# sdrobert/pydrobert-speech

Hardware: AMD Instinct MI355X
Metric: frames/s (whole node) + HBM-roofline %, 40-mel fbank 16kHz 25/10ms (higher is better)
Workload: dtype f32

## Files before the change

pydrobert-speech_amd/csrc/pds_internal.h:

```cpp
#pragma once
#include <hip/hip_runtime.h>
#include <stdint.h>

#include <exception>
#include <new>
#include <string>

#include "../../include/pds_amd.h"

namespace pds {

void set_error(const std::string &msg);
int32_t hip_fail(hipError_t err, const char *what);

#define PDS_HIP(call)                                       \
  do {                                                      \
    hipError_t _e = (call);                                 \
    if (_e != hipSuccess) return pds::hip_fail(_e, #call);  \
  } while (0)

struct FastTables {
  int kind = 0;
  int n1 = 0, n2 = 0;
  int rows = 0;
  int num_cus = 0;
  float *d_window = nullptr;
  float *d_twiddle = nullptr;
  float *d_tw_special = nullptr;
  float *d_win_half = nullptr;
  float *d_tw_seed = nullptr;
  float *d_ell_w = nullptr;
  int32_t *d_ell_meta = nullptr;
  int32_t *d_ell_len = nullptr;
  int32_t *d_ell_woff = nullptr;
  int ell_wfloats = 0, ell_slots = 0;
  float *d_seg_w = nullptr;
  int32_t *d_seg_meta = nullptr;
  int seg_rounds = 0, seg_len = 0, seg_wfloats = 0, seg_meta_ints = 0;
  float *d_rs_w = nullptr;
  int32_t *d_rs_meta = nullptr;
  int rs_rounds = 0, rs_len = 0, rs_wfloats = 0;
  float *d_rsn_w = nullptr;
  int32_t *d_rsn_meta = nullptr;
  int rsn_rounds = 0, rsn_len = 0, rsn_wfloats = 0;
  int rs_eslot = -1;
  float *d_ms_w = nullptr;
  int32_t *d_ms_meta = nullptr;
  int ms_rounds = 0, ms_len = 0, ms_wfloats = 0, ms_meta_ints = 0, ms_slots = 0;
  long ms_reads = 0;
  int walk = 0;
  long rs_reads = 0, rs_cost = 0, ell_reads = 0, seg_reads = 0;
  float *d_mf_tab = nullptr;
  int mf_rows = 0;
};

}

struct pds_stft_plan {
  pds_stft_desc d;
  int device = 0;
  int num_bins = 0;
  float *d_window_f32 = nullptr;
  double *d_window_f64 = nullptr;
  int32_t *d_row_ptr = nullptr;
// ... 128 lines not shown
```

pydrobert-speech_amd/csrc/stft_fast.hip:

```cpp
#include "stft_wave_launch.h"

namespace pds {

#if PDS_STAMPS
unsigned long long *g_stamp_buf = nullptr;
extern "C" __attribute__((visibility("default"))) void pds_debug_set_stamp_buffer(unsigned long long *d_buf) {
  g_stamp_buf = d_buf;
}
#endif

extern "C" __attribute__((visibility("default"))) int32_t pds_build_experiments(void) { return PDS_EXPERIMENTS ? 1 : 0; }

bool fast_has_f64in(const pds_stft_plan *plan) { return plan->fast.kind && fast_f64in_kind(plan->fast.kind); }

bool fast_has_fused_cmvn(const pds_stft_plan *plan) {
  const FastTables &ft = plan->fast;
  return ft.kind && ft.n2 == 16 && ((ft.n1 == 64 && ft.walk != 0) || (ft.n1 == 32 && (ft.walk == 1 || ft.walk == 3)));
}

bool fast_has_fused_deltas(const pds_stft_plan *plan) {
  const FastTables &ft = plan->fast;
  return ft.kind && fast_deltas_kind(ft.kind) && ft.rsn_rounds >= 1 && ft.rsn_rounds <= 2 &&
         (!plan->d.include_energy || ft.rs_eslot >= 0);
}
// ... 157 lines not shown
        first[j] = (pstr - longest) & ~3;
      if (first[j] < 0) return PDS_OK;
      ell_meta[(size_t)sl * n2 + j] = first[j] | ((f + 1) << 16);
      if (f < 0) continue;
      for (int q = row_ptr[f]; q < row_ptr[f + 1]; ++q) {
        const int t = col[q] - first[j];
        if (t < 0 || t >= longest) return PDS_OK;
        ell_w[(size_t)ell_woff[sl] + (size_t)j * wstride + t] = (float)val[q];
      }
    }
  }
  if (ell_w.empty()) ell_w.assign(4, 0.0f);
  ft.ell_wfloats = (int)ell_w.size();
  ft.ell_slots = slots;
  int32_t rc = PDS_OK;
  const int groups = 64 / n2;
  bool dense_bank = false;
  long dense_reads = 0;
  if ((n2 == 16 || (pow2 && n2 >= 32)) && d.num_filts > 0 && d.num_filts <= 65535) {
    long ell_reads = 0;
    for (int sl = 0; sl < slots; ++sl) ell_reads += 2L * (ell_len[sl] / 4);
    ft.ell_reads = ell_reads;
    const int free_slots = (wave_area_floats(n1, n2) - groups * pstr) / groups;
    int best_len = 0, best_rounds = 0;
    long best_reads = 0, any_reads = 0;
    const char *only_len = std::getenv("PDS_SEG_LEN");
    for (int len : {16, 32, 64}) {
      if (only_len && std::atoi(only_len) != len) continue;
      long nseg = 0;
      for (int f = 0; f < d.num_filts; ++f) nseg += (span(f) + len - 1) / len;
// ... 33 lines not shown
          if (first < 0) ok = false;
          seg_meta[slot] = first;
          for (int q = row_ptr[f]; q < row_ptr[f + 1]; ++q) {
            if (col[q] < base + k * len || col[q] >= base + (k + 1) * len) continue;
            const int t = col[q] - first;
            if (t < 0 || t >= len) ok = false; else seg_w[(size_t)slot * wstride + t] = (float)val[q];
          }
        }
      }
      if (ok) {
        ft.seg_reads = best_reads;
        ft.seg_rounds = best_rounds;
        ft.seg_len = len;
        ft.seg_wfloats = (int)seg_w.size();
        ft.seg_meta_ints = (int)seg_meta.size();
        if (rc == PDS_OK) rc = upload(&ft.d_seg_w, seg_w.data(), seg_w.size());
        if (rc == PDS_OK) rc = upload(&ft.d_seg_meta, seg_meta.data(), seg_meta.size());
      }
    }
  }
  if (n2 == 16 && rc == PDS_OK) {
    RsegTables rs;
    const int area_floats = wave_area_floats(n1, n2);
    if (build_rseg(d.num_filts, row_ptr, col, val, N / 2 + 1, area_floats / 4, 8, rs)) {
      ft.rs_rounds = rs.rounds;
      ft.rs_len = rs.seg_len;
      ft.rs_wfloats = (int)rs.w.size();
      ft.rs_reads = rs.reads_per_lane();
      ft.rs_cost = rs.cost;
      RsegTables rn;
      ft.rs_eslot = -1;
      if (rc == PDS_OK && fast_deltas_kind(N) && build_rseg(d.num_filts, row_ptr, col, val, N / 2 + 1, area_floats / 4, 2, rn, true)) {
        ft.rsn_rounds = rn.rounds;
        ft.rsn_len = rn.seg_len;
        ft.rsn_wfloats = (int)rn.w.size();
        for (size_t at = 0; at < rn.meta.size() && ft.rs_eslot < 0; ++at)
          if ((rn.meta[at] >> 16) == 0) ft.rs_eslot = (int)at;
        rc = upload(&ft.d_rsn_w, rn.w.data(), rn.w.size());
        if (rc == PDS_OK) rc = upload(&ft.d_rsn_meta, rn.meta.data(), rn.meta.size());
      }
      if (rc == PDS_OK) rc = upload(&ft.d_rs_w, rs.w.data(), rs.w.size());
      if (rc == PDS_OK) rc = upload(&ft.d_rs_meta, rs.meta.data(), rs.meta.size());
    }
  }
  if (n2 == 16 && pow2 && rc == PDS_OK && dense_bank) {
    MsegTables ms;
    const int area_floats = wave_area_floats(n1, n2);
    const int max_slots = (area_floats - 4 * pstr) / 16;
    if (build_mseg(d.num_filts, row_ptr, col, val, pstr, max_slots, ms)) {
      ft.ms_rounds = ms.rounds;
      ft.ms_slots = ms.slots;
      ft.ms_len = ms.seg_len;
      ft.ms_wfloats = (int)ms.w.size();
      ft.ms_meta_ints = (int)ms.meta.size();
      ft.ms_reads = ms.reads_per_lane();
      rc = upload(&ft.d_ms_w, ms.w.data(), ms.w.size());
      if (rc == PDS_OK) rc = upload(&ft.d_ms_meta, ms.meta.data(), ms.meta.size());
    }
  }
  {
    const char *force = std::getenv("PDS_STFT_WALK");
    ft.walk = ft.seg_rounds > 0 ? 1 : 0;
    const bool ms_stands_in = ft.walk == 0 && dense_bank && ft.ms_rounds > 0 && N >= PDS_MSEG_MIN_N;
    const long other = ft.walk == 1 ? ft.seg_reads : ms_stands_in ? dense_reads : ft.ell_reads;
    if (ft.rs_rounds > 0 && 10 * ft.rs_reads <= 7 * other) ft.walk = 2;
    if (force && std::strcmp(force, "ell") == 0) ft.walk = 0;
    if (force && std::strcmp(force, "seg") == 0) ft.walk = ft.seg_rounds > 0 ? 1 : 0;
    if (force && std::strcmp(force, "rseg") == 0) ft.walk = ft.rs_rounds > 0 ? 2 : ft.walk;
    if ((ft.walk == 1 || (ft.walk == 0 && ms_stands_in)) && ft.ms_rounds > 0 && N >= PDS_MSEG_MIN_N && !force) ft.walk = 3;
    if (force && std::strcmp(force, "mseg") == 0 && ft.ms_rounds > 0) ft.walk = 3;
    if (std::getenv("PDS_DEBUG_PLAN"))
      std::fprintf(stderr,
                   "pds plan N=%d filters=%d: ell slots %d reads %ld | seg rounds %d len %d reads %ld | rseg rounds %d "
                   "len %d reads %ld cost %ld | mseg rounds %d len %d reads %ld -> walk %d\n",
                   N, d.num_filts, ft.ell_slots, ft.ell_reads, ft.seg_rounds, ft.seg_len, ft.seg_reads, ft.rs_rounds,
                   ft.rs_len, ft.rs_reads, ft.rs_cost, ft.ms_rounds, ft.ms_len, ft.ms_reads, ft.walk);
  }
  if (rc == PDS_OK) rc = upload(&ft.d_ell_w, ell_w.data(), ell_w.size());
  if (rc == PDS_OK) rc = upload(&ft.d_ell_meta, ell_meta.data(), ell_meta.size());
  if (rc == PDS_OK) rc = upload(&ft.d_ell_len, ell_len.data(), ell_len.size());
  if (rc == PDS_OK) rc = upload(&ft.d_ell_woff, ell_woff.data(), ell_woff.size());
  if (rc == PDS_OK) rc = upload(&ft.d_window, win.data(), win.size());
  if (rc == PDS_OK) rc = upload(&ft.d_twiddle, tw.data(), tw.size());
  if (((n1 == 32 || n1 == 64) && n2 == 16) || lean_geometry(n1, n2)) {
    std::vector<float> wh(win), seed((size_t)n2 * 6);
    for (float &v : wh) v *= PDS_RDFT_DIT ? 1.0f : 0.5f;
    const int mult[3] = {1, 4, n1 / 4};
    for (int r = 0; r < n2; ++r)
      for (int j = 0; j < 3; ++j) {
        const double ang = -2.0 * M_PI * (double)((r * mult[j]) % N) / (double)N;
        seed[((size_t)r * 3 + j) * 2 + 0] = (float)std::cos(ang);
        seed[((size_t)r * 3 + j) * 2 + 1] = (float)std::sin(ang);
      }
    if (rc == PDS_OK) rc = upload(&ft.d_win_half, wh.data(), wh.size());
    if (rc == PDS_OK) rc = upload(&ft.d_tw_seed, seed.data(), seed.size());
  }
  std::vector<float> tws((size_t)n2 * 2);
  for (int r = 0; r < n2; ++r) {
    const double ang = -2.0 * M_PI * (double)r / (double)(2 * n2);
    tws[2 * r] = (float)std::cos(ang);
    tws[2 * r + 1] = (float)std::sin(ang);
  }
  if (rc == PDS_OK) rc = upload(&ft.d_tw_special, tws.data(), tws.size());
  {
    const char *front = PDS_EXPERIMENTS ? std::getenv("PDS_STFT_FRONT") : nullptr;
    const int rows = (d.frame_length + n2 - 1) / n2;
    int bucket = 0;
    for (int b : {20, 25, 28, 30, 32})
      if (!bucket && rows <= b) bucket = b;
    MfmaFrontTables mt;
    if (rc == PDS_OK && n1 == 32 && n2 == 16 && bucket && front && std::strcmp(front, "mfma") == 0 &&
        build_mfma_front(n1, bucket, d.frame_length, window, mt)) {
      std::vector<float> image;
      image.reserve(mt.words());
      image.insert(image.end(), mt.win.begin(), mt.win.end());
      for (int32_t v : mt.off) {
        float f;
        std::memcpy(&f, &v, sizeof f);
// ... 10 lines not shown
  if (rc != PDS_OK) return rc;
  hipDeviceProp_t prop;
  PDS_HIP(hipGetDeviceProperties(&prop, plan->device));
  ft.num_cus = prop.multiProcessorCount;
  ft.n1 = n1;
  ft.n2 = n2;
  ft.rows = (d.frame_length + n2 - 1) / n2;
  ft.kind = d.dft_size;
  return PDS_OK;
}

void fast_tables_destroy(pds_stft_plan *plan) {
  FastTables &ft = plan->fast;
  (void)hipFree(ft.d_window);
  (void)hipFree(ft.d_twiddle);
  (void)hipFree(ft.d_tw_special);
  (void)hipFree(ft.d_win_half);
  (void)hipFree(ft.d_tw_seed);
  (void)hipFree(ft.d_mf_tab);
  (void)hipFree(ft.d_rs_w);
  (void)hipFree(ft.d_ms_w);
  (void)hipFree(ft.d_ms_meta);
  (void)hipFree(ft.d_rsn_w);
  (void)hipFree(ft.d_rsn_meta);
  (void)hipFree(ft.d_rs_meta);
  (void)hipFree(ft.d_seg_w);
  (void)hipFree(ft.d_seg_meta);
  (void)hipFree(ft.d_ell_w);
  (void)hipFree(ft.d_ell_meta);
  (void)hipFree(ft.d_ell_len);
  (void)hipFree(ft.d_ell_woff);
  ft = FastTables();
}

}
```

pydrobert-speech_amd/csrc/stft_switches.h:

```cpp
#pragma once
namespace pds {

#ifndef PDS_PRIO_PACK
#define PDS_PRIO_PACK 0x103212
#endif
#if PDS_PRIO_PACK == 0xffffff
#define PDS_PHASE(i) __builtin_amdgcn_sched_barrier(0)
#else
#define PDS_PHASE(i) do { if (PDS_PRIO_PACK >= 0) __builtin_amdgcn_s_setprio(((PDS_PRIO_PACK) >> (4 * (i))) & 3); } while (0)
#endif
#ifndef PDS_ABLATE
#define PDS_ABLATE 0
#endif
#ifndef PDS_STAMPS
#define PDS_STAMPS 0
#endif
#if PDS_STAMPS
extern unsigned long long *g_stamp_buf;
#define PDS_STAMP(i, drain)                                               \
  do {                                                                    \
    if (PDS_STAMPS == 2) break;                                           \
    __builtin_amdgcn_sched_barrier(0);                                    \
    if (drain) asm volatile("s_waitcnt vmcnt(0)" ::: "memory");           \
    const unsigned long long now_ = __builtin_readcyclecounter();         \
// ... 6 lines not shown
#endif
#ifndef PDS_SEG_DEEP_N
#define PDS_SEG_DEEP_N 1024
#endif
#ifndef PDS_ELL_DEEP_N
#define PDS_ELL_DEEP_N 4096
#endif
#ifndef PDS_MSEG_MIN_N
#define PDS_MSEG_MIN_N 1024
#endif
#ifndef PDS_PAIR_SPLIT
#define PDS_PAIR_SPLIT 1
#endif
#ifndef PDS_N4096_MINW
#define PDS_N4096_MINW 2
#endif
#ifndef PDS_FAST_PROLOGUE
#define PDS_FAST_PROLOGUE 1
#endif
#ifndef PDS_MSEG_RED4
#define PDS_MSEG_RED4 1
#endif
#ifndef PDS_FILTER_UNROLL
#define PDS_FILTER_UNROLL 2
#endif
#ifndef PDS_EXPERIMENTS
#define PDS_EXPERIMENTS 0
#endif
#ifndef PDS_RDFT_DIT
#define PDS_RDFT_DIT (!PDS_EXPERIMENTS)
#endif
#ifndef PDS_WINDOW_CONTRACT
#define PDS_WINDOW_CONTRACT 0
// ... 48 lines not shown
```

pydrobert-speech_amd/csrc/stft_wave_kernel.h:

```cpp
#pragma once
#include <algorithm>
#include <atomic>
#include <cmath>
#include <cstdio>
#include <cstdlib>
#include <cstring>
#include <type_traits>
#include <vector>

#include "fft_inlane.h"
#include "mfma_front.h"
#include "rseg_tables.h"
#include "mseg_tables.h"
#include "pds_internal.h"

#include "stft_switches.h"

namespace pds {

__device__ __forceinline__ void keep_alive(float v) { asm volatile("" ::"v"(v)); }

struct FastParams {
  const void *sig;
  const int64_t *offsets, *lengths, *nframes, *row_off;
  void *out;
  int64_t out_stride;
  const float *win_lane;
  const float2 *tw_lane;
  const float2 *tw_special;
  const float *win_half;
  const float2 *tw_seed;
  const float *ell_w;
  const int32_t *ell_meta;
  const int32_t *ell_len;
  const int32_t *ell_woff;
  int ell_wfloats, ell_slots, ell_meta_pad, ell_meta_ints;
  int seg_rounds, seg_len, num_filts;
  int L, S, pad_left, include_energy, use_power, use_log;
  float log_floor, inv_L, preemph;
  double preemph_d;
  int chunks_per_utt, num_utts;
  int waves;
  int area_f;
  unsigned waves_rcp;
  int lds_ticket_off;
  int dyn;
  const float *mf_tab;
  unsigned long long *stamps;
// ... 85 lines not shown
  static constexpr int RSF = N2 + 4;
  static constexpr int XROWS = TWOPASS ? N2 : COLS;
  static constexpr int EXCH_F2 = wave_area_floats(N1, N2) / 2;
  static_assert(LEAN ? GROUPS * XROWS * RSF <= EXCH_F2 * 2 : GROUPS * XROWS * RS <= EXCH_F2, "the exchange must fit the wave's area");
  static_assert(!LEAN || (CPL == 1 && N2 >= 32), "lean form: one column per lane");
  static constexpr int PSTR = ((NB + 1 + 15) / 32) * 32 + 16;
  static_assert(GROUPS * PSTR <= EXCH_F2 * 2, "P must fit over the exchange area");
  static constexpr int XMIN_F = LEAN ? GROUPS * XROWS * RSF : GROUPS * XROWS * RS * 2;
  static constexpr int GCH = XMIN_F / 64 < NROWS ? XMIN_F / 64 : NROWS;
  static_assert(N % 2 == 0 && CPL >= 1 && N2 <= 64 && (RS * 8) % 16 == 0, "geometry");
  static_assert(inl::is_pow2(N1) ? (FULL || N2 == 2 * COLS) : 600 % N1 == 0,
                "in-lane DFT sizes: 2^k, or a divisor of 600");
  static_assert(NROWS <= N1 && NROWS > 0, "rows");
};

constexpr int USLOTS = 4;

typedef float f32x4 __attribute__((ext_vector_type(4)));

template <int N1, int N2, int NROWS, int MAXWAVES, int MINW, bool ELL_LDS, bool PRE, int SEG = 0, int MF = 0,
          bool RSG = false, typename TIN = float, typename TOUT = float, int DLT = 0, bool STR = false, bool PF = false>
__global__ __launch_bounds__(MAXWAVES * 64, MINW) void stft_wave_kernel(const FastParams p) {
  static_assert(!PF || (DLT == 0 && !STR && MF == 0 && !PRE && std::is_same<TIN, float>::value && (N1 == 32 || N1 == 64) && N2 == 16),
                "prefetch: 16-lane power-of-two geometries, float32 samples, round-robin scheduling");
  constexpr bool STRETCH = DLT > 0 || STR;
  static_assert(!(STR && DLT > 0), "stretch scheduling is part of the fused-deltas launches already");
  static_assert(DLT == 0 || (DLT == 2 && N2 == 16 && RSG && std::is_same<TOUT, float>::value && MF == 0),
                "fused deltas: row-segment walk, float32 features");
  static_assert(MF == 0 || std::is_same<TIN, float>::value, "matrix-pipe front end: float32 samples");
  static_assert(std::is_same<TIN, float>::value || std::is_same<TIN, double>::value || std::is_same<TIN, int16_t>::value, "samples: float32, float64 or int16");
  using G = WaveGeom<N1, N2, NROWS>;
  constexpr int N = G::N, COLS = G::COLS, NREG = G::NREG, RS = G::RS, NB = G::NB, PSTR = G::PSTR;
  constexpr int MSLOTS = 2 * MF + 1;
  static_assert(MF == 0 || (N2 == 16 && N1 == 32 && MF == mfma_front_steps(NROWS)), "matrix-pipe front end: 32 x 16");
  static_assert(MF == 0 || 4 * MSLOTS * 64 <= G::EXCH_F2 * 2, "edge-frame gather reuses the exchange area");
  constexpr int NBP = (NB + 3) / 4 * 4;
  static_assert(!RSG || (G::GROUPS == 4 && ELL_LDS && !SEG && (NBP + 1) * 4 <= G::EXCH_F2 * 2),
                "row-segment walk: four frames per wave, tables in LDS");
  extern __shared__ __attribute__((aligned(16))) float smem[];
  const int lane = threadIdx.x & 63;
  const int wave = __builtin_amdgcn_readfirstlane(threadIdx.x >> 6);
  const int g = lane / N2, r = lane % N2;
  constexpr bool F64S = std::is_same<TIN, double>::value;
  constexpr bool PAIR = F64S && N2 == 16 && MF == 0;
  const int rho = PAIR ? ((r & 7) * 2 + (r >> 3)) : r;
  constexpr int LOADSPAN = PAIR ? (NROWS + 1) / 2 * 32 : NROWS * N2;
  [[maybe_unused]] const unsigned long long st_entry = PDS_STAMPS ? __builtin_readcyclecounter() : 0;
  float *wbase = smem + wave * p.area_f;
  [[maybe_unused]] double *wstat = reinterpret_cast<double *>(smem + p.lds_stat_off) + wave * (2 * p.stat_cs);
  constexpr bool STATS = STR && G::GROUPS == 4 && (SEG != 0 || (RSG && MINW <= 2));
  [[maybe_unused]] const bool stats_on = STATS && p.stat_part != nullptr;
  [[maybe_unused]] auto stat_add4 = [&](const int col, const float (&v)[4], const int nf) {
    double t1 = 0.0, t2 = 0.0;
#pragma unroll
    for (int q = 0; q < 4; ++q)
      if (q < nf) {
        const double d = (double)v[q];
        t1 += d;
        t2 = fma(d, d, t2);
      }
    wstat[col] += t1;
    wstat[p.stat_cs + col] += t2;
  };
  float2 *exch = reinterpret_cast<float2 *>(wbase) + g * G::XROWS * RS;
  [[maybe_unused]] float *xf = wbase + g * (G::XROWS * G::RSF);
  float *Pg = wbase + g * PSTR;
  const int nthreads = p.waves * 64;
  float2 *sw_lds = reinterpret_cast<float2 *>(smem + p.waves * p.area_f);
  int *meta_lds = reinterpret_cast<int *>(sw_lds + N2);
  float *ellw_lds = reinterpret_cast<float *>(meta_lds + p.ell_meta_pad);
  constexpr bool TWCHAIN = (PF && PDS_PF_TW == 1) || (PAIR && (N1 == 32 || N1 == 64)) || (PDS_DLT_CHAIN && DLT > 0 && N1 == 32 && N2 == 16) || G::LEAN ||
                           (N1 == 64 && N2 == 16 && (SEG == 2 || PDS_LEAN_1024));
  constexpr bool WINLDS = PF && PDS_PF_WIN == 1;
  constexpr bool WINUSE = G::LEAN || (N1 == 64 && N2 == 16 && (SEG == 2 || PDS_LEAN_1024));
  constexpr int WSTR = win_table_stride(NROWS);
  [[maybe_unused]] float *win_lds = ellw_lds + (ELL_LDS ? p.ell_wfloats : 0);
  if constexpr (WINLDS || WINUSE) {
    const float *wsrc = TWCHAIN ? p.win_half : p.win_lane;
    for (int i = threadIdx.x; i < N2 * WSTR; i += p.waves * 64) {
      const int rr = i / WSTR, k = i - rr * WSTR;
      win_lds[i] = k < NROWS ? wsrc[rr * N1 + k] : 0.0f;
    }
  }
  if (threadIdx.x < N2) sw_lds[threadIdx.x] = p.tw_special[threadIdx.x];
  constexpr bool DYN = PDS_DYN && !STRETCH && !PF;
  [[maybe_unused]] int *ticket_lds = reinterpret_cast<int *>(smem + p.lds_ticket_off);
  if constexpr (DYN) {
    if (threadIdx.x == 0) *ticket_lds = p.waves;
  }
  if constexpr (STR && G::GROUPS == 4 && (SEG != 0 || (RSG && MINW <= 2))) {
    if (p.stat_part) {
      double *z = reinterpret_cast<double *>(smem + p.lds_stat_off);
      for (int i = threadIdx.x; i < p.waves * 2 * p.stat_cs; i += p.waves * 64) z[i] = 0.0;
    }
  }
  if constexpr (RSG) {
    int4 *rec_lds = reinterpret_cast<int4 *>(meta_lds);
    for (int i = threadIdx.x; i < p.seg_rounds * 64; i += nthreads) {
      const int m = p.ell_meta[i], f = (m >> 16) - 1;
      rec_lds[i] = make_int4((m & 0x3fff) * 16, __float_as_int((m & (1 << 14)) ? 1.0f : 0.0f),
                             __float_as_int((m & (1 << 15)) ? 1.0f : 0.0f),
                             f >= 0 ? ((p.include_energy ? 1 : 0) + f) * (int)sizeof(TOUT) : -1);
    }
  } else {
    for (int i = threadIdx.x; i < p.ell_meta_pad; i += nthreads)
      meta_lds[i] = i < p.ell_meta_ints ? p.ell_meta[i] : 0;
  }
#if PDS_FAST_PROLOGUE
  static_assert((G::EXCH_F2 * 2) % 4 == 0, "wave areas are zeroed 16 bytes at a time");
  if constexpr (ELL_LDS) {
    const float4 *src4 = reinterpret_cast<const float4 *>(p.ell_w);
    float4 *dst4 = reinterpret_cast<float4 *>(ellw_lds);
    for (int i = threadIdx.x; i < (p.ell_wfloats >> 2); i += nthreads) dst4[i] = src4[i];
  }
  {
    float4 *z4 = reinterpret_cast<float4 *>(smem);
    for (int i = threadIdx.x; i < p.waves * (p.area_f / 4); i += nthreads) z4[i] = make_float4(0.0f, 0.0f, 0.0f, 0.0f);
  }
#else
  if constexpr (ELL_LDS)
    for (int i = threadIdx.x; i < p.ell_wfloats; i += nthreads) ellw_lds[i] = p.ell_w[i];
  for (int i = threadIdx.x; i < p.waves * p.area_f; i += nthreads) smem[i] = 0.0f;
#endif
  __syncthreads();

  [[maybe_unused]] float win[(MF || WINLDS || WINUSE) ? 1 : NROWS];
  [[maybe_unused]] float twr[(MF || TWCHAIN) ? 1 : COLS], twi[(MF || TWCHAIN) ? 1 : COLS];
  [[maybe_unused]] float sd[6] = {0.0f, 0.0f, 0.0f, 0.0f, 0.0f, 0.0f};
  [[maybe_unused]] float mwin[MSLOTS], mare[MF + 1], maim[MF + 1], mtwr[4], mtwi[4];
  [[maybe_unused]] unsigned moff[MSLOTS];
  if constexpr (MF > 0) {
    const float *tab = p.mf_tab;
#pragma unroll
    for (int sl = 0; sl < MSLOTS; ++sl) {
      mwin[sl] = tab[sl * 64 + lane];
      moff[sl] = (unsigned)reinterpret_cast<const int *>(tab)[(MSLOTS + sl) * 64 + lane] * 4u;
    }
#pragma unroll
    for (int t = 0; t <= MF; ++t) {
      mare[t] = tab[(3 * MSLOTS + t) * 64 + lane];
      maim[t] = tab[(3 * MSLOTS + MF + 1 + t) * 64 + lane];
    }
#pragma unroll
    for (int v = 0; v < 4; ++v) {
      const float2 t = reinterpret_cast<const float2 *>(tab + (3 * MSLOTS + 2 * (MF + 1)) * 64)[v * 64 + lane];
// ... 10 lines not shown
#pragma unroll
      for (int j = 0; j < 3; ++j) {
        const float2 t = p.tw_seed[rho * 3 + j];
        sd[2 * j] = t.x;
        sd[2 * j + 1] = t.y;
      }
    } else {
#pragma unroll
      for (int k1 = 1; k1 <= NREG; ++k1) {
        const float2 t = p.tw_lane[rho * COLS + k1];
        twr[k1] = t.x;
        twi[k1] = t.y;
      }
    }
  }
  [[maybe_unused]] float pfv[PF ? NROWS : 1];
  [[maybe_unused]] float wl[WINLDS ? NROWS : 1];
  [[maybe_unused]] auto read_window = [&]() {
    if constexpr (WINLDS) {
      const float4 *w4 = reinterpret_cast<const float4 *>(win_lds + rho * WSTR);
#pragma unroll
      for (int j = 0; j < (NROWS + 3) / 4; ++j) {
        const float4 w = w4[j];
        const float wv[4] = {w.x, w.y, w.z, w.w};
#pragma unroll
        for (int u = 0; u < 4; ++u)
          if (4 * j + u < NROWS) wl[4 * j + u] = wv[u];
      }
    }
  };
  read_window();
  [[maybe_unused]] bool pf_ready = false;
  [[maybe_unused]] const int pf_lane = __mul24(g, p.S) + r;
  const int L = p.L, S = p.S;
  const bool use_power = p.use_power != 0;
  const int col0 = p.include_energy ? 1 : 0;

  int b = 0;
  int wg = blockIdx.x;
#ifndef PDS_NO_XCD_MAP
  if ((gridDim.x & 7) == 0) wg = (wg & 7) * (gridDim.x >> 3) + (wg >> 3);
#endif
  int chunk = wg * p.waves + wave;
  if constexpr (!STRETCH) {
    while (chunk >= p.chunks_per_utt && b < p.num_utts) {
      chunk -= p.chunks_per_utt;
// ... 127 lines not shown
                const float4 val = *reinterpret_cast<const float4 *>(stage + q * WS + 4 * l);
                F4 o = {val.x, val.y, val.z, val.w};
                *reinterpret_cast<F4 *>(orow + (int64_t)q * p.out_stride + 4 * l) = o;
              }
          }
        }
      }
      if (tail) {
        const int q = tail == 1 ? lane : tail == 2 ? lane >> 1 : (lane * 11) >> 5;
        const int jj = lane - q * tail;
        if (q < fh && q < 4) orow[(int64_t)q * p.out_stride + 4 * full + jj] = stage[q * WS + 4 * full + jj];
      }
    }
    wave_sync();
  };
  [[maybe_unused]] unsigned long long st_acc[8] = {0, 0, 0, 0, 0, 0, 0, 0};
  [[maybe_unused]] unsigned long long st_prev = PDS_STAMPS ? __builtin_readcyclecounter() : 0;
  [[maybe_unused]] const unsigned long long st_loop = st_prev;
  while (STRETCH || b < p.num_utts) {
    if constexpr (STRETCH) {
      if (!piece_open) {
        if (left <= 0) break;
        nfr = (int)load_const(p.nframes + b);
        const int chunks_b = (nfr + G::GROUPS - 1) / G::GROUPS;
        if (e_lo >= chunks_b) {
          ++b;
          e_lo = 0;
          continue;
        }
        n = (int)load_const(p.lengths + b);
// ... 1174 lines not shown
```

pydrobert-speech_amd/csrc/stft_wave_launch.h:

```cpp
#pragma once
#include "stft_wave_kernel.h"

namespace pds {


constexpr bool fast_f64in_kind(int n) { return n == 256 || n == 512 || n == 1024 || n == 2048; }

constexpr bool fast_deltas_kind(int n) { return n == 512 || n == 1024; }


template <int N1, int N2, int NROWS, int MINW>
int32_t launch_wave(const pds_stft_plan *plan, const BatchArgs &a) {
  using G = WaveGeom<N1, N2, NROWS>;
#ifndef PDS_DLT_MINW
#define PDS_DLT_MINW 3
#endif
  constexpr int DMINW = (N1 == 64 && N2 == 16) ? 2 : MINW > PDS_DLT_MINW ? PDS_DLT_MINW : MINW;
  constexpr int CU_WAVES_STFT = 4 * MINW;
  constexpr int F64_MINW = (N1 == 64 && N2 == 16) ? 2 : MINW, F64_WAVES = 4 * F64_MINW;
  const int CU_WAVES = a.dl_K > 0 ? 4 * DMINW : a.in_f64 ? F64_WAVES : CU_WAVES_STFT;
  const FastTables &ft = plan->fast;
  FastParams p;
  p.sig = a.d_signal;
  p.offsets = a.d_offsets;
  p.lengths = a.d_lengths;
  p.nframes = a.d_nframes;
  p.row_off = a.d_row_off;
  p.out = a.d_out;
  p.out_stride = a.out_stride;
  p.win_lane = ft.d_window;
  p.tw_lane = (const float2 *)ft.d_twiddle;
  p.tw_special = (const float2 *)ft.d_tw_special;
  constexpr bool LEAN_ALL = G::LEAN || (PDS_LEAN_1024 && N1 == 64 && N2 == 16);
  p.win_half = LEAN_ALL ? ft.d_win_half : nullptr;
  p.tw_seed = LEAN_ALL ? (const float2 *)ft.d_tw_seed : nullptr;
  p.ell_w = ft.d_ell_w;
  p.ell_meta = ft.d_ell_meta;
  p.ell_len = ft.d_ell_len;
  p.ell_woff = ft.d_ell_woff;
  p.ell_wfloats = ft.ell_wfloats;
  p.ell_slots = ft.ell_slots;
  p.L = plan->d.frame_length;
  p.S = plan->d.frame_shift;
  p.pad_left = a.pad_left;
  p.include_energy = plan->d.include_energy;
  p.use_power = plan->d.use_power;
  p.use_log = plan->d.use_log;
  p.log_floor = (float)plan->d.log_floor;
  p.inv_L = 1.0f / (float)plan->d.frame_length;
  p.num_utts = a.B;
  const int64_t chunks = (a.max_frames + G::GROUPS - 1) / G::GROUPS;
  if (chunks * a.B > 0x7fffffff || chunks > 0x3fffffff || a.out_stride * G::GROUPS > (a.out_f64 ? 0x0fffffff : 0x1fffffff) ||
// ... 34 lines not shown
  constexpr bool MSEG3 = N1 == 64 && N2 == 16;
  constexpr int MS_WAVES = MSEG3 ? 12 : 4 * MINW, MS_MINW = MSEG3 ? 3 : MINW;
  static_assert(!MSEG3 || !PDS_LEAN_1024 || MINW == 3, "the 64 x 16 geometry is instantiated for three waves per SIMD (stft_geoms.def)");
  const bool pf_ok = (PDS_EXPERIMENTS || PF_PRODUCT) && PFG && !pre && !a.in_f64 && !a.in_i16 && !a.stretch && a.dl_K == 0 &&
                     ft.d_win_half && ft.d_tw_seed && !(pf_env && pf_env[0] == '0');
  constexpr int PF_WSTR = ((NROWS + 3) & ~3) % 8 == 4 ? ((NROWS + 3) & ~3) : ((NROWS + 3) & ~3) + 4;
  const size_t pf_extra = (PDS_PF_WIN == 1) ? (size_t)N2 * PF_WSTR * 4 : 0;
  const size_t lean_extra = LEAN_ALL ? (size_t)N2 * win_table_stride(NROWS) * 4 : 0;
  const size_t mseg3_extra = LEAN_ALL ? 0 : (size_t)N2 * win_table_stride(NROWS) * 4;
  constexpr bool MSG = G::GROUPS == 4 && inl::is_pow2(N1);
  constexpr bool SEGOK = G::GROUPS == 4 || (inl::is_pow2(N1) && N2 >= 32);
  for (int cand = (G::GROUPS == 4) ? (dl ? 2 : ft.walk) : (SEGOK && ft.walk == 1 ? 1 : 0); cand >= 0 && !in_lds; --cand) {
    if (cand == 3 && (!MSG || ft.ms_rounds == 0 || pre || a.in_f64 || a.in_i16)) continue;
    if ((cand == 2 && !dl && ft.rs_rounds == 0) || (cand == 1 && (ft.seg_rounds == 0 || pre || a.in_f64 || a.in_i16))) continue;
    const int meta_ints = cand == 3 ? ft.ms_meta_ints : cand == 2 ? (dl ? ft.rsn_rounds : ft.rs_rounds) * 64 : cand == 1 ? ft.seg_meta_ints : ft.ell_slots * N2;
    const int meta_pad = cand == 2 ? meta_ints * 4 : (std::max(meta_ints, USLOTS * N2) + 3) / 4 * 4;
    const size_t fixed = (size_t)N2 * 8 + (size_t)meta_pad * 4 + (cand == 2 && pf_ok ? pf_extra : 0) + lean_extra +
                         (cand == 3 && MSEG3 ? mseg3_extra : 0);
    const size_t table_bytes = (size_t)(cand == 3 ? ft.ms_wfloats : cand == 2 ? (dl ? ft.rsn_wfloats : ft.rs_wfloats) : cand == 1 ? ft.seg_wfloats : ft.ell_wfloats) * 4;
    if (cand == 1 && (size_t)G::GROUPS * G::PSTR * 4 + (size_t)ft.seg_rounds * 64 * 4 * G::GROUPS > per_wave) continue;
    if (cand == 3 && (size_t)G::GROUPS * G::PSTR * 4 + (size_t)ft.ms_slots * 64 > per_wave) continue;
    const size_t area_c = (cand == 3 && MSEG3)
                              ? std::max((size_t)G::XMIN_F * 4, (size_t)G::GROUPS * G::PSTR * 4 + (size_t)ft.ms_slots * 64)
                              : per_wave;
    const int ms_shapes[5][2] = {{12, 1}, {11, 1}, {10, 1}, {9, 1}, {8, 1}};
    const int (*try_shapes)[2] = (cand == 3 && MSEG3) ? ms_shapes : shapes;
    for (int si = 0; si < ((cand == 3 && MSEG3) ? 5 : 4); ++si) {
      const int *shape = try_shapes[si];
      if (shape[0] * (area_c + stat_pw) + fixed + table_bytes + 48 <= lds_cu / shape[1]) {
        waves = shape[0];
        wgs_per_cu = shape[1];
        in_lds = true;
        area_bytes = area_c;
        break;
      }
    }
    p.ell_meta_pad = meta_pad;
    p.ell_meta_ints = meta_ints;
    if (in_lds && cand == 3) {
      p.ell_w = ft.d_ms_w;
      p.ell_meta = ft.d_ms_meta;
      p.ell_wfloats = ft.ms_wfloats;
      p.seg_rounds = ft.ms_rounds;
      p.seg_len = ft.ms_len;
    } else if (in_lds && cand == 1) {
      p.ell_w = ft.d_seg_w;
      p.ell_meta = ft.d_seg_meta;
      p.ell_wfloats = ft.seg_wfloats;
      p.seg_rounds = ft.seg_rounds;
      p.seg_len = ft.seg_len;
    } else if (in_lds && cand == 2) {
      p.ell_w = dl ? ft.d_rsn_w : ft.d_rs_w;
      p.ell_meta = dl ? ft.d_rsn_meta : ft.d_rs_meta;
      p.ell_wfloats = dl ? ft.rsn_wfloats : ft.rs_wfloats;
      p.seg_rounds = dl ? ft.rsn_rounds : ft.rs_rounds;
      p.seg_len = dl ? ft.rsn_len : ft.rs_len;
    }
    if (in_lds) walk = cand;
  }
#ifdef PDS_FORCE_WAVES
  if (in_lds && PDS_FORCE_WAVES <= CU_WAVES / 2) waves = PDS_FORCE_WAVES, wgs_per_cu = 2;
#endif
  const size_t fixed = (size_t)N2 * 8 + (size_t)p.ell_meta_pad * 4 + (walk == 2 && in_lds && pf_ok ? pf_extra : 0) + lean_extra +
                       (walk == 3 && in_lds && MSEG3 ? mseg3_extra : 0);
  const size_t table_bytes = (size_t)p.ell_wfloats * 4;
  if (a.in_i16 && !in_lds) {
    set_error("stft_batch_i16in: not served for this plan (filter table outside LDS)");
    return PDS_ERR_INVALID;
  }
  if (pre && !in_lds) return launch_stft_generic_f32(plan, a);
  p.preemph = (float)a.preemph;
  p.preemph_d = a.preemph;
  p.waves = waves;
  p.mf_tab = ft.d_mf_tab;
#if PDS_STAMPS
  p.stamps = g_stamp_buf;
#else
  p.stamps = nullptr;
#endif
  p.area_f = (int)(area_bytes / 4);
// ... 205 lines not shown
```

Baseline: 4.070 billion.

## Prebuild contiguous LDS table images on host and stream them in one copy

Precomputes on the host a single contiguous image holding the special twiddles, the metadata (with RSG walk records already expanded) and the filter weights for each walk variant. The kernel prologue then becomes one float4 copy instead of several separate loops, including the per-entry record decoding. The copy is split so the first chunk's global loads are issued early and their stores to LDS are deferred until after the lane-constant setup, so load latency overlaps other prologue work. In exchange it uses extra device memory for the duplicated images, including a separate f64-output variant, and the prologue ordering is more intricate.

Measured after the change: 4.064 billion, median of 2. About the same (-0.1%).

```diff
diff --git a/pydrobert-speech_amd/csrc/pds_internal.h b/pydrobert-speech_amd/csrc/pds_internal.h
--- a/pydrobert-speech_amd/csrc/pds_internal.h
+++ b/pydrobert-speech_amd/csrc/pds_internal.h
@@ -26,28 +26,19 @@
   int num_cus = 0;
   float *d_window = nullptr;
   float *d_twiddle = nullptr;
-  float *d_tw_special = nullptr;
   float *d_win_half = nullptr;
   float *d_tw_seed = nullptr;
-  float *d_ell_w = nullptr;
-  int32_t *d_ell_meta = nullptr;
   int32_t *d_ell_len = nullptr;
   int32_t *d_ell_woff = nullptr;
   int ell_wfloats = 0, ell_slots = 0;
-  float *d_seg_w = nullptr;
-  int32_t *d_seg_meta = nullptr;
   int seg_rounds = 0, seg_len = 0, seg_wfloats = 0, seg_meta_ints = 0;
-  float *d_rs_w = nullptr;
-  int32_t *d_rs_meta = nullptr;
   int rs_rounds = 0, rs_len = 0, rs_wfloats = 0;
-  float *d_rsn_w = nullptr;
-  int32_t *d_rsn_meta = nullptr;
   int rsn_rounds = 0, rsn_len = 0, rsn_wfloats = 0;
   int rs_eslot = -1;
-  float *d_ms_w = nullptr;
-  int32_t *d_ms_meta = nullptr;
   int ms_rounds = 0, ms_len = 0, ms_wfloats = 0, ms_meta_ints = 0, ms_slots = 0;
   long ms_reads = 0;
+  float *d_img_ell = nullptr, *d_img_seg = nullptr, *d_img_rs = nullptr, *d_img_rs64 = nullptr, *d_img_rsn = nullptr,
+        *d_img_ms = nullptr;
   int walk = 0;
   long rs_reads = 0, rs_cost = 0, ell_reads = 0, seg_reads = 0;
   float *d_mf_tab = nullptr;
diff --git a/pydrobert-speech_amd/csrc/stft_fast.hip b/pydrobert-speech_amd/csrc/stft_fast.hip
--- a/pydrobert-speech_amd/csrc/stft_fast.hip
+++ b/pydrobert-speech_amd/csrc/stft_fast.hip
@@ -195,6 +195,13 @@
   ft.ell_wfloats = (int)ell_w.size();
   ft.ell_slots = slots;
   int32_t rc = PDS_OK;
+  struct Image {
+    float **dst;
+    int walk, meta_ints;
+    std::vector<int32_t> meta;
+    std::vector<float> w;
+  };
+  std::vector<Image> images;
   const int groups = 64 / n2;
   bool dense_bank = false;
   long dense_reads = 0;
@@ -258,8 +265,7 @@
         ft.seg_len = len;
         ft.seg_wfloats = (int)seg_w.size();
         ft.seg_meta_ints = (int)seg_meta.size();
-        if (rc == PDS_OK) rc = upload(&ft.d_seg_w, seg_w.data(), seg_w.size());
-        if (rc == PDS_OK) rc = upload(&ft.d_seg_meta, seg_meta.data(), seg_meta.size());
+        images.push_back({&ft.d_img_seg, 1, ft.seg_meta_ints, seg_meta, seg_w});
       }
     }
   }
@@ -280,11 +286,15 @@
         ft.rsn_wfloats = (int)rn.w.size();
         for (size_t at = 0; at < rn.meta.size() && ft.rs_eslot < 0; ++at)
           if ((rn.meta[at] >> 16) == 0) ft.rs_eslot = (int)at;
-        rc = upload(&ft.d_rsn_w, rn.w.data(), rn.w.size());
-        if (rc == PDS_OK) rc = upload(&ft.d_rsn_meta, rn.meta.data(), rn.meta.size());
-      }
-      if (rc == PDS_OK) rc = upload(&ft.d_rs_w, rs.w.data(), rs.w.size());
-      if (rc == PDS_OK) rc = upload(&ft.d_rs_meta, rs.meta.data(), rs.meta.size());
+        std::vector<int32_t> rec;
+        build_walk_records(rn.meta.data(), (int)rn.meta.size(), d.include_energy != 0, (int)sizeof(float), rec);
+        images.push_back({&ft.d_img_rsn, 2, (int)rn.meta.size(), rec, rn.w});
+      }
+      std::vector<int32_t> rec;
+      build_walk_records(rs.meta.data(), (int)rs.meta.size(), d.include_energy != 0, (int)sizeof(float), rec);
+      images.push_back({&ft.d_img_rs, 2, (int)rs.meta.size(), rec, rs.w});
+      build_walk_records(rs.meta.data(), (int)rs.meta.size(), d.include_energy != 0, (int)sizeof(double), rec);
+      images.push_back({&ft.d_img_rs64, 2, (int)rs.meta.size(), rec, rs.w});
     }
   }
   if (n2 == 16 && pow2 && rc == PDS_OK && dense_bank) {
@@ -298,8 +308,7 @@
       ft.ms_wfloats = (int)ms.w.size();
       ft.ms_meta_ints = (int)ms.meta.size();
       ft.ms_reads = ms.reads_per_lane();
-      rc = upload(&ft.d_ms_w, ms.w.data(), ms.w.size());
-      if (rc == PDS_OK) rc = upload(&ft.d_ms_meta, ms.meta.data(), ms.meta.size());
+      images.push_back({&ft.d_img_ms, 3, ft.ms_meta_ints, ms.meta, ms.w});
     }
   }
   {
@@ -320,8 +329,8 @@
                    N, d.num_filts, ft.ell_slots, ft.ell_reads, ft.seg_rounds, ft.seg_len, ft.seg_reads, ft.rs_rounds,
                    ft.rs_len, ft.rs_reads, ft.rs_cost, ft.ms_rounds, ft.ms_len, ft.ms_reads, ft.walk);
   }
-  if (rc == PDS_OK) rc = upload(&ft.d_ell_w, ell_w.data(), ell_w.size());
-  if (rc == PDS_OK) rc = upload(&ft.d_ell_meta, ell_meta.data(), ell_meta.size());
+  ell_meta.resize((size_t)slots * n2);
+  images.push_back({&ft.d_img_ell, 0, slots * n2, ell_meta, ell_w});
   if (rc == PDS_OK) rc = upload(&ft.d_ell_len, ell_len.data(), ell_len.size());
   if (rc == PDS_OK) rc = upload(&ft.d_ell_woff, ell_woff.data(), ell_woff.size());
   if (rc == PDS_OK) rc = upload(&ft.d_window, win.data(), win.size());
@@ -345,7 +354,12 @@
     tws[2 * r] = (float)std::cos(ang);
     tws[2 * r + 1] = (float)std::sin(ang);
   }
-  if (rc == PDS_OK) rc = upload(&ft.d_tw_special, tws.data(), tws.size());
+  for (const Image &im : images) {
+    std::vector<float> image;
+    build_lds_image(n2, tws.data(), im.meta.data(), (int)im.meta.size(), walk_meta_pad(im.walk, im.meta_ints, n2),
+                    im.w.data(), (int)im.w.size(), image);
+    if (rc == PDS_OK) rc = upload(im.dst, image.data(), image.size());
+  }
   {
     const char *front = PDS_EXPERIMENTS ? std::getenv("PDS_STFT_FRONT") : nullptr;
     const int rows = (d.frame_length + n2 - 1) / n2;
@@ -386,20 +400,15 @@
   FastTables &ft = plan->fast;
   (void)hipFree(ft.d_window);
   (void)hipFree(ft.d_twiddle);
-  (void)hipFree(ft.d_tw_special);
   (void)hipFree(ft.d_win_half);
   (void)hipFree(ft.d_tw_seed);
   (void)hipFree(ft.d_mf_tab);
-  (void)hipFree(ft.d_rs_w);
-  (void)hipFree(ft.d_ms_w);
-  (void)hipFree(ft.d_ms_meta);
-  (void)hipFree(ft.d_rsn_w);
-  (void)hipFree(ft.d_rsn_meta);
-  (void)hipFree(ft.d_rs_meta);
-  (void)hipFree(ft.d_seg_w);
-  (void)hipFree(ft.d_seg_meta);
-  (void)hipFree(ft.d_ell_w);
-  (void)hipFree(ft.d_ell_meta);
+  (void)hipFree(ft.d_img_ell);
+  (void)hipFree(ft.d_img_seg);
+  (void)hipFree(ft.d_img_rs);
+  (void)hipFree(ft.d_img_rs64);
+  (void)hipFree(ft.d_img_rsn);
+  (void)hipFree(ft.d_img_ms);
   (void)hipFree(ft.d_ell_len);
   (void)hipFree(ft.d_ell_woff);
   ft = FastTables();
diff --git a/pydrobert-speech_amd/csrc/stft_switches.h b/pydrobert-speech_amd/csrc/stft_switches.h
--- a/pydrobert-speech_amd/csrc/stft_switches.h
+++ b/pydrobert-speech_amd/csrc/stft_switches.h
@@ -44,9 +44,6 @@
 #endif
 #ifndef PDS_N4096_MINW
 #define PDS_N4096_MINW 2
-#endif
-#ifndef PDS_FAST_PROLOGUE
-#define PDS_FAST_PROLOGUE 1
 #endif
 #ifndef PDS_MSEG_RED4
 #define PDS_MSEG_RED4 1
diff --git a/pydrobert-speech_amd/csrc/stft_wave_kernel.h b/pydrobert-speech_amd/csrc/stft_wave_kernel.h
--- a/pydrobert-speech_amd/csrc/stft_wave_kernel.h
+++ b/pydrobert-speech_amd/csrc/stft_wave_kernel.h
@@ -12,6 +12,7 @@
 #include "mfma_front.h"
 #include "rseg_tables.h"
 #include "mseg_tables.h"
+#include "walk_records.h"
 #include "pds_internal.h"
 
 #include "stft_switches.h"
@@ -27,11 +28,10 @@
   int64_t out_stride;
   const float *win_lane;
   const float2 *tw_lane;
-  const float2 *tw_special;
+  const float *lds_img;
   const float *win_half;
   const float2 *tw_seed;
   const float *ell_w;
-  const int32_t *ell_meta;
   const int32_t *ell_len;
   const int32_t *ell_woff;
   int ell_wfloats, ell_slots, ell_meta_pad, ell_meta_ints;
@@ -147,7 +147,7 @@
   static_assert(NROWS <= N1 && NROWS > 0, "rows");
 };
 
-constexpr int USLOTS = 4;
+constexpr int USLOTS = kEllUnrolledSlots;
 
 typedef float f32x4 __attribute__((ext_vector_type(4)));
 
@@ -171,6 +171,9 @@
   static_assert(!RSG || (G::GROUPS == 4 && ELL_LDS && !SEG && (NBP + 1) * 4 <= G::EXCH_F2 * 2),
                 "row-segment walk: four frames per wave, tables in LDS");
   extern __shared__ __attribute__((aligned(16))) float smem[];
+  asm volatile("" ::"s"(p.lds_img), "s"(p.ell_meta_pad), "s"(p.ell_wfloats), "s"(p.waves),
+               "s"(p.area_f), "s"(p.win_lane), "s"(p.tw_lane), "s"(p.chunks_per_utt), "s"(p.num_utts), "s"(p.nframes),
+               "s"(p.lengths), "s"(p.offsets), "s"(p.row_off));
   const int lane = threadIdx.x & 63;
   const int wave = __builtin_amdgcn_readfirstlane(threadIdx.x >> 6);
   const int g = lane / N2, r = lane % N2;
@@ -199,23 +202,37 @@
   [[maybe_unused]] float *xf = wbase + g * (G::XROWS * G::RSF);
   float *Pg = wbase + g * PSTR;
   const int nthreads = p.waves * 64;
-  float2 *sw_lds = reinterpret_cast<float2 *>(smem + p.waves * p.area_f);
-  int *meta_lds = reinterpret_cast<int *>(sw_lds + N2);
-  float *ellw_lds = reinterpret_cast<float *>(meta_lds + p.ell_meta_pad);
+  float *tables_lds = smem + p.waves * p.area_f;
+  const WalkLdsLayout lds_at = walk_lds_layout(N2, p.ell_meta_pad, ELL_LDS ? p.ell_wfloats : 0);
+  float2 *sw_lds = reinterpret_cast<float2 *>(tables_lds + lds_at.tw_special);
+  int *meta_lds = reinterpret_cast<int *>(tables_lds + lds_at.meta);
+  float *ellw_lds = tables_lds + lds_at.weights;
   constexpr bool TWCHAIN = (PF && PDS_PF_TW == 1) || (PAIR && (N1 == 32 || N1 == 64)) || (PDS_DLT_CHAIN && DLT > 0 && N1 == 32 && N2 == 16) || G::LEAN ||
                            (N1 == 64 && N2 == 16 && (SEG == 2 || PDS_LEAN_1024));
   constexpr bool WINLDS = PF && PDS_PF_WIN == 1;
   constexpr bool WINUSE = G::LEAN || (N1 == 64 && N2 == 16 && (SEG == 2 || PDS_LEAN_1024));
   constexpr int WSTR = win_table_stride(NROWS);
-  [[maybe_unused]] float *win_lds = ellw_lds + (ELL_LDS ? p.ell_wfloats : 0);
+  [[maybe_unused]] float *win_lds = tables_lds + lds_at.window;
+  const int tid = threadIdx.x;
+  constexpr int TU = 1;
+  const int tab4 = (ELL_LDS ? lds_at.window : lds_at.weights) >> 2;
+  const float4 *tab_src4 = reinterpret_cast<const float4 *>(p.lds_img);
+  float4 *tab_dst4 = reinterpret_cast<float4 *>(tables_lds);
+  float4 tab_v[TU];
+  [[maybe_unused]] float win_v = 0.0f;
+  [[maybe_unused]] auto win_src = [&](const int i) {
+    const float *wsrc = TWCHAIN ? p.win_half : p.win_lane;
+    const int rr = i / WSTR, k = i - rr * WSTR;
+    return k < NROWS ? wsrc[rr * N1 + k] : 0.0f;
+  };
+#pragma unroll
+  for (int u = 0; u < TU; ++u) {
+    tab_v[u] = make_float4(0.0f, 0.0f, 0.0f, 0.0f);
+    if (tid + u * nthreads < tab4) tab_v[u] = tab_src4[tid + u * nthreads];
+  }
   if constexpr (WINLDS || WINUSE) {
-    const float *wsrc = TWCHAIN ? p.win_half : p.win_lane;
-    for (int i = threadIdx.x; i < N2 * WSTR; i += p.waves * 64) {
-      const int rr = i / WSTR, k = i - rr * WSTR;
-      win_lds[i] = k < NROWS ? wsrc[rr * N1 + k] : 0.0f;
-    }
+    if (tid < N2 * WSTR) win_v = win_src(tid);
   }
-  if (threadIdx.x < N2) sw_lds[threadIdx.x] = p.tw_special[threadIdx.x];
   constexpr bool DYN = PDS_DYN && !STRETCH && !PF;
   [[maybe_unused]] int *ticket_lds = reinterpret_cast<int *>(smem + p.lds_ticket_off);
   if constexpr (DYN) {
@@ -227,41 +244,19 @@
       for (int i = threadIdx.x; i < p.waves * 2 * p.stat_cs; i += p.waves * 64) z[i] = 0.0;
     }
   }
-  if constexpr (RSG) {
-    int4 *rec_lds = reinterpret_cast<int4 *>(meta_lds);
-    for (int i = threadIdx.x; i < p.seg_rounds * 64; i += nthreads) {
-      const int m = p.ell_meta[i], f = (m >> 16) - 1;
-      rec_lds[i] = make_int4((m & 0x3fff) * 16, __float_as_int((m & (1 << 14)) ? 1.0f : 0.0f),
-                             __float_as_int((m & (1 << 15)) ? 1.0f : 0.0f),
-                             f >= 0 ? ((p.include_energy ? 1 : 0) + f) * (int)sizeof(TOUT) : -1);
-    }
-  } else {
-    for (int i = threadIdx.x; i < p.ell_meta_pad; i += nthreads)
-      meta_lds[i] = i < p.ell_meta_ints ? p.ell_meta[i] : 0;
-  }
-#if PDS_FAST_PROLOGUE
   static_assert((G::EXCH_F2 * 2) % 4 == 0, "wave areas are zeroed 16 bytes at a time");
-  if constexpr (ELL_LDS) {
-    const float4 *src4 = reinterpret_cast<const float4 *>(p.ell_w);
-    float4 *dst4 = reinterpret_cast<float4 *>(ellw_lds);
-    for (int i = threadIdx.x; i < (p.ell_wfloats >> 2); i += nthreads) dst4[i] = src4[i];
-  }
   {
     float4 *z4 = reinterpret_cast<float4 *>(smem);
     for (int i = threadIdx.x; i < p.waves * (p.area_f / 4); i += nthreads) z4[i] = make_float4(0.0f, 0.0f, 0.0f, 0.0f);
   }
-#else
-  if constexpr (ELL_LDS)
-    for (int i = threadIdx.x; i < p.ell_wfloats; i += nthreads) ellw_lds[i] = p.ell_w[i];
-  for (int i = threadIdx.x; i < p.waves * p.area_f; i += nthreads) smem[i] = 0.0f;
-#endif
-  __syncthreads();
 
   [[maybe_unused]] float win[(MF || WINLDS || WINUSE) ? 1 : NROWS];
   [[maybe_unused]] float twr[(MF || TWCHAIN) ? 1 : COLS], twi[(MF || TWCHAIN) ? 1 : COLS];
   [[maybe_unused]] float sd[6] = {0.0f, 0.0f, 0.0f, 0.0f, 0.0f, 0.0f};
   [[maybe_unused]] float mwin[MSLOTS], mare[MF + 1], maim[MF + 1], mtwr[4], mtwi[4];
   [[maybe_unused]] unsigned moff[MSLOTS];
+  constexpr bool CONST_EARLY = !(STR && RSG && N1 == 32 && N2 == 16 && NROWS == 25 && MINW == 4);
+  auto load_lane_constants = [&]() {
   if constexpr (MF > 0) {
     const float *tab = p.mf_tab;
 #pragma unroll
@@ -302,6 +297,8 @@
       }
     }
   }
+  };
+  if constexpr (CONST_EARLY) load_lane_constants();
   [[maybe_unused]] float pfv[PF ? NROWS : 1];
   [[maybe_unused]] float wl[WINLDS ? NROWS : 1];
   [[maybe_unused]] auto read_window = [&]() {
@@ -317,7 +314,6 @@
       }
     }
   };
-  read_window();
   [[maybe_unused]] bool pf_ready = false;
   [[maybe_unused]] const int pf_lane = __mul24(g, p.S) + r;
   const int L = p.L, S = p.S;
@@ -475,6 +471,27 @@
     }
     wave_sync();
   };
+#pragma unroll
+  for (int u = 0; u < TU; ++u)
+    if (tid + u * nthreads < tab4) tab_dst4[tid + u * nthreads] = tab_v[u];
+  for (int i = tid + TU * nthreads; i < tab4; i += nthreads) tab_dst4[i] = tab_src4[i];
+  if constexpr (WINLDS || WINUSE) {
+    if (tid < N2 * WSTR) win_lds[tid] = win_v;
+    for (int i = tid + nthreads; i < N2 * WSTR; i += nthreads) win_lds[i] = win_src(i);
+  }
+  __syncthreads();
+  if constexpr (!CONST_EARLY) load_lane_constants();
+  if constexpr (MF == 0 && CONST_EARLY) {
+    if constexpr (!WINLDS && !WINUSE) {
+#pragma unroll
+      for (int n1 = 0; n1 < NROWS; ++n1) asm volatile("" : "+v"(win[n1]));
+    }
+    if constexpr (!TWCHAIN) {
+#pragma unroll
+      for (int k1 = 1; k1 <= NREG; ++k1) asm volatile("" : "+v"(twr[k1]), "+v"(twi[k1]));
+    }
+  }
+  read_window();
   [[maybe_unused]] unsigned long long st_acc[8] = {0, 0, 0, 0, 0, 0, 0, 0};
   [[maybe_unused]] unsigned long long st_prev = PDS_STAMPS ? __builtin_readcyclecounter() : 0;
   [[maybe_unused]] const unsigned long long st_loop = st_prev;
diff --git a/pydrobert-speech_amd/csrc/stft_wave_launch.h b/pydrobert-speech_amd/csrc/stft_wave_launch.h
--- a/pydrobert-speech_amd/csrc/stft_wave_launch.h
+++ b/pydrobert-speech_amd/csrc/stft_wave_launch.h
@@ -30,12 +30,10 @@
   p.out_stride = a.out_stride;
   p.win_lane = ft.d_window;
   p.tw_lane = (const float2 *)ft.d_twiddle;
-  p.tw_special = (const float2 *)ft.d_tw_special;
   constexpr bool LEAN_ALL = G::LEAN || (PDS_LEAN_1024 && N1 == 64 && N2 == 16);
   p.win_half = LEAN_ALL ? ft.d_win_half : nullptr;
   p.tw_seed = LEAN_ALL ? (const float2 *)ft.d_tw_seed : nullptr;
-  p.ell_w = ft.d_ell_w;
-  p.ell_meta = ft.d_ell_meta;
+  p.lds_img = ft.d_img_ell;
   p.ell_len = ft.d_ell_len;
   p.ell_woff = ft.d_ell_woff;
   p.ell_wfloats = ft.ell_wfloats;
@@ -100,8 +98,8 @@
     if (cand == 3 && (!MSG || ft.ms_rounds == 0 || pre || a.in_f64 || a.in_i16)) continue;
     if ((cand == 2 && !dl && ft.rs_rounds == 0) || (cand == 1 && (ft.seg_rounds == 0 || pre || a.in_f64 || a.in_i16))) continue;
     const int meta_ints = cand == 3 ? ft.ms_meta_ints : cand == 2 ? (dl ? ft.rsn_rounds : ft.rs_rounds) * 64 : cand == 1 ? ft.seg_meta_ints : ft.ell_slots * N2;
-    const int meta_pad = cand == 2 ? meta_ints * 4 : (std::max(meta_ints, USLOTS * N2) + 3) / 4 * 4;
-    const size_t fixed = (size_t)N2 * 8 + (size_t)meta_pad * 4 + (cand == 2 && pf_ok ? pf_extra : 0) + lean_extra +
+    const int meta_pad = walk_meta_pad(cand, meta_ints, N2);
+    const size_t fixed = walk_lds_bytes(N2, meta_pad, 0, 0) + (cand == 2 && pf_ok ? pf_extra : 0) + lean_extra +
                          (cand == 3 && MSEG3 ? mseg3_extra : 0);
     const size_t table_bytes = (size_t)(cand == 3 ? ft.ms_wfloats : cand == 2 ? (dl ? ft.rsn_wfloats : ft.rs_wfloats) : cand == 1 ? ft.seg_wfloats : ft.ell_wfloats) * 4;
     if (cand == 1 && (size_t)G::GROUPS * G::PSTR * 4 + (size_t)ft.seg_rounds * 64 * 4 * G::GROUPS > per_wave) continue;
@@ -124,20 +122,17 @@
     p.ell_meta_pad = meta_pad;
     p.ell_meta_ints = meta_ints;
     if (in_lds && cand == 3) {
-      p.ell_w = ft.d_ms_w;
-      p.ell_meta = ft.d_ms_meta;
+      p.lds_img = ft.d_img_ms;
       p.ell_wfloats = ft.ms_wfloats;
       p.seg_rounds = ft.ms_rounds;
       p.seg_len = ft.ms_len;
     } else if (in_lds && cand == 1) {
-      p.ell_w = ft.d_seg_w;
-      p.ell_meta = ft.d_seg_meta;
+      p.lds_img = ft.d_img_seg;
       p.ell_wfloats = ft.seg_wfloats;
       p.seg_rounds = ft.seg_rounds;
       p.seg_len = ft.seg_len;
     } else if (in_lds && cand == 2) {
-      p.ell_w = dl ? ft.d_rsn_w : ft.d_rs_w;
-      p.ell_meta = dl ? ft.d_rsn_meta : ft.d_rs_meta;
+      p.lds_img = dl ? ft.d_img_rsn : a.out_f64 ? ft.d_img_rs64 : ft.d_img_rs;
       p.ell_wfloats = dl ? ft.rsn_wfloats : ft.rs_wfloats;
       p.seg_rounds = dl ? ft.rsn_rounds : ft.rs_rounds;
       p.seg_len = dl ? ft.rsn_len : ft.rs_len;
@@ -147,9 +142,10 @@
 #ifdef PDS_FORCE_WAVES
   if (in_lds && PDS_FORCE_WAVES <= CU_WAVES / 2) waves = PDS_FORCE_WAVES, wgs_per_cu = 2;
 #endif
-  const size_t fixed = (size_t)N2 * 8 + (size_t)p.ell_meta_pad * 4 + (walk == 2 && in_lds && pf_ok ? pf_extra : 0) + lean_extra +
+  const size_t fixed = walk_lds_bytes(N2, p.ell_meta_pad, 0, 0) + (walk == 2 && in_lds && pf_ok ? pf_extra : 0) + lean_extra +
                        (walk == 3 && in_lds && MSEG3 ? mseg3_extra : 0);
   const size_t table_bytes = (size_t)p.ell_wfloats * 4;
+  p.ell_w = p.lds_img + walk_lds_layout(N2, p.ell_meta_pad, 0).weights;
   if (a.in_i16 && !in_lds) {
     set_error("stft_batch_i16in: not served for this plan (filter table outside LDS)");
     return PDS_ERR_INVALID;
diff --git a/pydrobert-speech_amd/csrc/walk_records.h b/pydrobert-speech_amd/csrc/walk_records.h
--- /dev/null
+++ b/pydrobert-speech_amd/csrc/walk_records.h
@@ -0,0 +1,55 @@
+#pragma once
+#include <cstddef>
+#include <cstdint>
+#include <cstring>
+#include <vector>
+
+namespace pds {
+
+constexpr int kWalkRecordWords = 4;
+
+constexpr int kEllUnrolledSlots = 4;
+
+constexpr int walk_meta_pad(int walk, int meta_ints, int n2) {
+  return walk == 2 ? meta_ints * kWalkRecordWords
+                   : ((meta_ints > kEllUnrolledSlots * n2 ? meta_ints : kEllUnrolledSlots * n2) + 3) / 4 * 4;
+}
+
+struct WalkLdsLayout {
+  int tw_special = 0, meta = 0, weights = 0, window = 0;
+};
+constexpr WalkLdsLayout walk_lds_layout(int n2, int meta_pad, int wfloats) {
+  return WalkLdsLayout{0, 2 * n2, 2 * n2 + meta_pad, 2 * n2 + meta_pad + wfloats};
+}
+constexpr size_t walk_lds_bytes(int n2, int meta_pad, int wfloats, int window_floats) {
+  return (size_t)(walk_lds_layout(n2, meta_pad, wfloats).window + window_floats) * 4;
+}
+
+inline void build_lds_image(int n2, const float *tw_special, const int32_t *meta, int meta_ints, int meta_pad,
+                            const float *w, int wfloats, std::vector<float> &image) {
+  const WalkLdsLayout at = walk_lds_layout(n2, meta_pad, wfloats);
+  image.assign((size_t)at.window, 0.0f);
+  std::memcpy(image.data() + at.tw_special, tw_special, sizeof(float) * 2 * (size_t)n2);
+  std::memcpy(image.data() + at.meta, meta, sizeof(int32_t) * (size_t)meta_ints);
+  std::memcpy(image.data() + at.weights, w, sizeof(float) * (size_t)wfloats);
+}
+
+inline void build_walk_records(const int32_t *meta, int entries, bool include_energy, int feature_bytes,
+                               std::vector<int32_t> &rec) {
+  rec.assign((size_t)entries * kWalkRecordWords, 0);
+  const float one = 1.0f, zero = 0.0f;
+  int32_t one_bits, zero_bits;
+  std::memcpy(&one_bits, &one, sizeof one_bits);
+  std::memcpy(&zero_bits, &zero, sizeof zero_bits);
+  for (int i = 0; i < entries; ++i) {
+    const int32_t m = meta[i];
+    const int f = (m >> 16) - 1;
+    int32_t *r = rec.data() + (size_t)i * kWalkRecordWords;
+    r[0] = (m & 0x3fff) * 16;
+    r[1] = (m & (1 << 14)) ? one_bits : zero_bits;
+    r[2] = (m & (1 << 15)) ? one_bits : zero_bits;
+    r[3] = f >= 0 ? ((include_energy ? 1 : 0) + f) * feature_bytes : -1;
+  }
+}
+
+}
```
